# Drehrumbum/viterbi.dll

Measured on AMD Instinct MI355X. Metric: decoded Mbit/s per GPU on batched 768-bit DAB FIC frames; bit-exact vs AVX2 ref, higher is better.
Workload: dtype u8

## Files before the change

viterbi.dll_amd/csrc/rs_dev.h:

```cpp
#pragma once
#include "vit_internal.h"

namespace {

constexpr int NN = 255;
constexpr int NROOTS = 10;
constexpr int PADN = 135;
constexpr int NCW = 120, NMSG = 110;
constexpr int RS_THREADS = 256;
constexpr int ATO_ZERO = 512;
constexpr int ATO_SIZE = 768;
#ifndef COOP_MAX3
#define COOP_MAX3 12
#endif
#ifndef COOP_MAX5
#define COOP_MAX5 28
#endif

struct GfTables {
    uint8_t ato[ATO_SIZE];
    uint8_t iof[256];
};
constexpr GfTables make_tables() {
    GfTables t{};
    uint8_t alpha[256] = {};
    int sr = 1;
    t.iof[0] = NN;
    for (int i = 0; i < NN; i++) {
        t.iof[sr] = (uint8_t)i;
        alpha[i] = (uint8_t)sr;
        sr <<= 1;
        if (sr & 256) sr ^= 285;
        sr &= NN;
    }
    for (int i = 0; i < ATO_ZERO; i++) t.ato[i] = alpha[i % 255];
    return t;
}
__constant__ GfTables g_gf = make_tables();

struct QuadTable {
    uint8_t q[256];
};
constexpr QuadTable make_quad_table() {
    const GfTables t = make_tables();
    QuadTable Q{};
    for (int y = 2; y < 256; y++) {
        const int y2 = t.ato[(2 * t.iof[y]) % 255];
        const int c = y2 ^ y;
        if (Q.q[c] == 0) Q.q[c] = (uint8_t)y;
    }
    return Q;
}

#ifndef RS_LFSR2
#define RS_LFSR2 1
#endif
constexpr int NIB_TABLES = RS_LFSR2 ? 4 : 2;
struct NibTable {
    uint32_t w[NIB_TABLES * 16 * 4];
};
constexpr NibTable make_nib_table() {
    const GfTables t = make_tables();
    uint8_t g[NROOTS + 1] = {1};
    int deg = 0;
    for (int i = 0; i < NROOTS; i++) {
        const uint8_t root = t.ato[i];
        uint8_t ng[NROOTS + 1] = {};
        for (int j = 0; j <= deg; j++) {
            ng[j + 1] ^= g[j];
            if (g[j]) ng[j] ^= t.ato[t.iof[g[j]] + t.iof[root]];
        }
        deg++;
        for (int j = 0; j <= deg; j++) g[j] = ng[j];
    }
    NibTable G{};
    for (int half = 0; half < 2; half++)
        for (int n = 1; n < 16; n++) {
            const int x = half ? n << 4 : n;
            for (int j = 0; j < NROOTS; j++) {
                const uint32_t prod = g[j] ? t.ato[t.iof[x] + t.iof[g[j]]] : 0u;
                G.w[(half * 16 + n) * 4 + (j < 8 ? j / 4 : 3)] |= prod << (8 * (j % 4));
            }
        }
#if RS_LFSR2
    for (int half = 0; half < 2; half++)
        for (int n = 1; n < 16; n++) {
            const int x = half ? n << 4 : n;
            for (int j = 0; j < NROOTS; j++) {
                uint8_t c = j ? g[j - 1] : 0;
                if (g[9] && g[j]) c ^= t.ato[t.iof[g[9]] + t.iof[g[j]]];
                const uint32_t prod = c ? t.ato[t.iof[x] + t.iof[c]] : 0u;
                G.w[((2 + half) * 16 + n) * 4 + (j < 8 ? j / 4 : 3)] |= prod << (8 * (j % 4));
            }
        }
#endif
    return G;
}
__constant__ NibTable g_nib = make_nib_table();
__constant__ QuadTable g_quad = make_quad_table();

constexpr int STEP_TERMS = 5;
struct StepTable {
    uint32_t w[STEP_TERMS * 256];
};
constexpr StepTable make_step_table() {
    const GfTables t = make_tables();
    StepTable S{};
    for (int j = 1; j <= STEP_TERMS; j++)
        for (int c = 1; c < 256; c++)
            for (int k = 1; k <= 4; k++) S.w[(j - 1) * 256 + c] |= (uint32_t)t.ato[t.iof[c] + j * k] << (8 * (k - 1));
    return S;
}
__constant__ StepTable g_step = make_step_table();

typedef uint32_t u32x4 __attribute__((ext_vector_type(4)));
#define LDS __attribute__((address_space(3)))
__device__ __forceinline__ uint32_t xor3(uint32_t a, uint32_t b, uint32_t c) { return __builtin_amdgcn_bitop3_b32(a, b, c, 0x96); }
__device__ __forceinline__ uint32_t mod255(uint32_t x) { return (x * 0x1010102u) >> 24; }
__device__ __forceinline__ uint32_t mod510(uint32_t x) { return x < x - NN ? x : x - NN; }

__device__ __forceinline__ int chien_log(const uint32_t (&lam)[NROOTS + 1], bool need, int deg_lambda, uint8_t* col,
                                         uint32_t stride, const uint8_t* __restrict__ ato) {
    uint32_t b[NROOTS + 1], live[NROOTS + 1];
#pragma unroll
    for (int j = 1; j <= NROOTS; j++) {
        live[j] = need && lam[j] != NN ? 0xFFu : 0u;
        b[j] = live[j] ? lam[j] : 0u;
    }
    bool searching = need;
    int count = 0;
    for (int i = 1; i <= NN; i++) {
        if (searching) {
            uint32_t q = 1;
#pragma unroll
            for (int j = 1; j <= NROOTS; j++) {
                b[j] += (uint32_t)j;
                b[j] = b[j] < (uint32_t)NN ? b[j] : b[j] - NN;
                q ^= ato[b[j]] & live[j];
            }
            if (q == 0) {
                col[(uint32_t)(NMSG + count) * stride] = (uint8_t)i;
                if (++count == deg_lambda) searching = false;
            }
        }
        if (!__any(searching)) break;
    }
    return count;
}

template <int D>
__device__ __forceinline__ int chien_quad(const uint32_t (&lam)[NROOTS + 1], bool need, uint8_t* col, uint32_t stride,
                                          const uint8_t* __restrict__ ato, const uint32_t* __restrict__ step) {
    static_assert(D <= STEP_TERMS, "step table");
    uint32_t adr[D + 1];
#pragma unroll
    for (int j = 1; j <= D; j++) adr[j] = need && lam[j] != NN ? (uint32_t)ato[lam[j]] << 2 : 0u;
    int count = 0;
    for (int blk = 0; blk < 8; blk++) {
        uint32_t m = 0;
#pragma unroll
        for (int it = 0; it < 8; it++) {
            uint32_t q = 0x01010101u;
#pragma unroll
            for (int j = 1; j <= D; j++) {
                const uint32_t t =
                    *reinterpret_cast<const uint32_t*>(reinterpret_cast<const uint8_t*>(step) + (j - 1) * 1024 + adr[j]);
                q ^= t;
                adr[j] = (t >> 22) & 0x3FCu;
            }
            const uint32_t z = ~(((q & 0x7F7F7F7Fu) + 0x7F7F7F7Fu) | q | 0x7F7F7F7Fu);
            m = (m >> 1) | z;
        }
        if (blk == 7) m &= 0x7FFFFFFFu;
        if (__any(m != 0)) {
            while (m) {
                const uint32_t bit = (uint32_t)__ffs((int)m) - 1u;
                m &= m - 1u;
                col[(uint32_t)(NMSG + count) * stride] = (uint8_t)(32u * blk + 4u * (bit & 7u) + (bit >> 3) + 1u);
                count++;
            }
        }
    }
    return count;
}

template <int D>
__device__ __forceinline__ void chien_wave(const uint32_t (&lam)[NROOTS + 1], bool need, bool failed, int deg_lambda,
                                           uint32_t sfid, int& count, bool& dropped, uint8_t* cwbase, uint32_t coloff,
                                           uint32_t stride, const uint8_t* __restrict__ ato,
                                           const uint32_t* __restrict__ step) {
    static_assert(D <= STEP_TERMS, "step table");
    const uint32_t lane = __lane_id();
    uint32_t e[D + 1], lgz[D + 1];
#pragma unroll
    for (int j = 1; j <= D; j++) {
        e[j] = mod255(4u * (uint32_t)j * lane);
        lgz[j] = lam[j] == (uint32_t)NN ? (uint32_t)ATO_ZERO : lam[j];
    }
    const uint32_t keep = lane == 63u ? 0x7FFFFFFFu : 0xFFFFFFFFu;
    const uint64_t failm = __ballot(failed);
    uint64_t work = __ballot(need) | failm;
    uint64_t gone = 0;
    while (work) {
        const int owner = __builtin_ctzll(work);
        work &= work - 1;
        bool fail = true;
        if (!((failm >> owner) & 1u)) {
            uint32_t q = 0x01010101u;
#pragma unroll
            for (int j = 1; j <= D; j++) {
                const uint32_t c = ato[(uint32_t)__builtin_amdgcn_readlane(lgz[j], owner) + e[j]];
                q ^= step[(j - 1) * 256 + c];
            }
            uint32_t z = ~(((q & 0x7F7F7F7Fu) + 0x7F7F7F7Fu) | q | 0x7F7F7F7Fu) & keep;
            uint8_t* ocol = cwbase + __builtin_amdgcn_readlane(coloff, owner);
            uint32_t found = 0;
            uint64_t hit;
            while ((hit = __ballot(z != 0)) != 0) {
                if (z) {
                    const uint32_t below =
                        __builtin_amdgcn_mbcnt_hi((uint32_t)(hit >> 32), __builtin_amdgcn_mbcnt_lo((uint32_t)hit, 0u));
                    const uint32_t k = ((uint32_t)__ffs((int)z) - 1u) >> 3;
                    ocol[__umul24(NMSG + found + below, stride)] = (uint8_t)(4u * lane + k + 1u);
                    z &= z - 1u;
                }
                found += (uint32_t)__popcll(hit);
            }
            if (lane == (uint32_t)owner) count = (int)found;
            fail = (int)found != __builtin_amdgcn_readlane(deg_lambda, owner);
        }
        if (fail) {
            const uint64_t later = __ballot(sfid == (uint32_t)__builtin_amdgcn_readlane(sfid, owner)) & ~((2ull << owner) - 1ull);
            work &= ~later;
            gone |= later;
        }
    }
    dropped = (gone >> lane) & 1u;
}

__device__ int rs_correct(uint32_t (&s)[NROOTS], bool err, uint32_t sfid, uint8_t* cwbase, uint32_t coloff,
                          uint32_t stride, const uint8_t* __restrict__ ato, const uint8_t* __restrict__ iof,
                          const uint8_t* __restrict__ qsol, const uint32_t* __restrict__ step) {
    uint8_t* const col = cwbase + coloff;
    uint32_t lam[NROOTS + 1];
#pragma unroll
    for (int i = 0; i <= NROOTS; i++) lam[i] = NN;
    int deg_lambda = 0;
    if (err) {
#pragma unroll
        for (int i = 0; i < NROOTS; i++) s[i] = iof[s[i]];

        uint32_t pl[NROOTS + 1], b[NROOTS + 1];
#pragma unroll
        for (int i = 0; i <= NROOTS; i++) { pl[i] = 0; b[i] = NN; }
        pl[0] = 1;
        lam[0] = 0;
        b[0] = 0;
        int el = 0;
        bool geo = s[0] != NN && s[1] != NN;
        const uint32_t lr = mod510(s[1] + NN - s[0]);
        uint32_t expect = s[1];
#pragma unroll
        for (int i = 2; i < NROOTS; i++) {
            expect = mod510(expect + lr);
            geo = geo && s[i] == expect;
        }
        const bool shortcut = __all(geo);
        if (shortcut) lam[1] = lr;
#pragma unroll
        for (int r = 1; r <= NROOTS; r++) {
            if (shortcut) break;
            uint32_t discr = 0;
#pragma unroll
            for (int i = 0; i < r; i++) {
                const bool term = lam[i] != NN && s[r - i - 1] != NN;
                if (__any(term)) {
                    if (term) discr ^= ato[lam[i] + s[r - i - 1]];
                }
            }
            discr = iof[discr];
            const bool zero = discr == NN;
            if (__any(!zero)) {
                const bool grow = !zero && 2 * el <= r - 1;
                uint32_t t[NROOTS + 1];
#pragma unroll
                for (int i = 0; i < r; i++) {
                    t[i + 1] = pl[i + 1];
                    if (!zero && b[i] != NN) t[i + 1] ^= ato[discr + b[i]];
                }
                if (grow) el = r - el;
#pragma unroll
                for (int i = r; i >= 0; i--) {
                    const uint32_t scaled = lam[i] == NN ? (uint32_t)NN : mod510(lam[i] + NN - discr);
                    const uint32_t shifted = i ? b[i - 1] : (uint32_t)NN;
                    b[i] = grow ? scaled : shifted;
                }
#pragma unroll
                for (int i = 1; i <= r; i++) {
                    pl[i] = zero ? pl[i] : t[i];
                    lam[i] = iof[pl[i]];
                }
            } else {
#pragma unroll
                for (int i = r; i > 0; i--) b[i] = b[i - 1];
                b[0] = NN;
            }
        }
#pragma unroll
        for (int i = 0; i <= NROOTS; i++)
            if (lam[i] != NN) deg_lambda = i;
    }
    int dmax = 0;
#pragma unroll
    for (int d = 1; d <= NROOTS; d++)
        if (__any(deg_lambda >= d)) dmax = d;
    dmax = __builtin_amdgcn_readfirstlane(dmax);

    uint32_t root[NROOTS];
#pragma unroll
    for (int k = 0; k < NROOTS; k++) root[k] = 0;
    int count = 0;
    if (deg_lambda == 1) {
        root[0] = (uint32_t)NN - lam[1];
        count = 1;
    } else if (dmax >= 2 && deg_lambda == 2) {
        if (lam[1] != NN) {
            const uint32_t y0 = qsol[ato[mod255(lam[2] + 2u * (NN - lam[1]))]];
            if (y0) {
                const uint32_t scale = lam[1] + NN - lam[2];
                uint32_t r0 = mod255(scale + iof[y0]), r1 = mod255(scale + iof[y0 ^ 1u]);
                r0 = r0 ? r0 : (uint32_t)NN;
                r1 = r1 ? r1 : (uint32_t)NN;
                root[0] = r0 < r1 ? r0 : r1;
                root[1] = r0 < r1 ? r1 : r0;
                count = 2;
            }
        } else {
            count = 1;
        }
    }
    bool dropped = false;
    if (dmax >= 3) {
        const bool need = deg_lambda >= 3;
        if (dmax <= STEP_TERMS) {
            const int heavy = __popcll(__ballot(need));
            if (heavy <= (dmax <= 3 ? COOP_MAX3 : COOP_MAX5)) {
                const bool failed = err && !need && deg_lambda != count;
                if (dmax <= 3) chien_wave<3>(lam, need, failed, deg_lambda, sfid, count, dropped, cwbase, coloff, stride, ato, step);
                else chien_wave<STEP_TERMS>(lam, need, failed, deg_lambda, sfid, count, dropped, cwbase, coloff, stride, ato, step);
            } else {
                const int found = dmax <= 3 ? chien_quad<3>(lam, need, col, stride, ato, step)
                                            : chien_quad<STEP_TERMS>(lam, need, col, stride, ato, step);
                if (need) count = found;
            }
        } else if (need) {
            count = chien_log(lam, need, deg_lambda, col, stride, ato);
        }
        if (need && !dropped) {
#pragma unroll
            for (int k = 0; k < NROOTS; k++)
                if (k < dmax && k < count) root[k] = col[(uint32_t)(NMSG + k) * stride];
        }
    }
    if (!err || dropped) return 0;
    if (deg_lambda != count) return -1;

    const int deg_omega = deg_lambda - 1;
    uint32_t om[NROOTS];
#pragma unroll
    for (int i = 0; i < NROOTS; i++) {
        om[i] = NN;
        if (i < dmax) {
            uint32_t tmp = 0;
#pragma unroll
            for (int j = 0; j <= i; j++)
                if (s[i - j] != NN && lam[j] != NN) tmp ^= ato[s[i - j] + lam[j]];
            om[i] = i <= deg_omega ? (uint32_t)iof[tmp] : (uint32_t)NN;
        }
    }
    const int top = (deg_lambda < NROOTS - 1 ? deg_lambda : NROOTS - 1) & ~1;
#pragma unroll
    for (int j = NROOTS - 1; j >= 0; j--) {
        if (j >= dmax) continue;
        const uint32_t rt = root[j];
        if (j < count && rt >= PADN + 1) {
            uint32_t num1 = 0;
#pragma unroll
            for (int i = 0; i < NROOTS; i++)
                if (i < dmax && i <= deg_omega && om[i] != NN) num1 ^= ato[mod255(om[i] + i * rt)];
            if (num1) {
                const uint32_t num2 = ato[NN - rt];
                uint32_t den = 0;
#pragma unroll
                for (int i = 0; i < NROOTS; i += 2)
                    if (i < dmax && i <= top && lam[i + 1] != NN) den ^= ato[mod255(lam[i + 1] + i * rt)];
                const uint32_t tmp = (uint32_t)iof[num1] + iof[num2] + (NN - iof[den]);
                col[(rt - 1 - PADN) * stride] ^= ato[mod255(tmp)];
            }
        }
    }
    return count;
}

__device__ int decode_rs(bool active, uint32_t sfid, uint8_t* cw, uint32_t tid, const uint8_t* __restrict__ ato,
                         const uint8_t* __restrict__ iof, const uint8_t* __restrict__ mulp,
                         const uint8_t* __restrict__ qsol, const uint32_t* __restrict__ step) {
    uint32_t s[NROOTS];
    uint32_t syn = 0;
    if (active) {
        const uint8_t* col = cw + tid;
        const uint32_t d0 = col[0];
#pragma unroll
        for (int i = 0; i < NROOTS; i++) s[i] = d0;
        for (int j = 1; j < NCW; j++) {
            const uint32_t d = col[j * RS_THREADS];
            s[0] ^= d;
#pragma unroll
            for (int i = 1; i < NROOTS; i++) s[i] = d ^ mulp[i * 256 + s[i]];
        }
#pragma unroll
        for (int i = 0; i < NROOTS; i++) syn |= s[i];
    }
    if (!__any(syn != 0)) return 0;
    return rs_correct(s, syn != 0, sfid, cw, tid, RS_THREADS, ato, iof, qsol, step);
}

__device__ int decode_rs_lfsr(bool active, uint32_t sfid, uint8_t* cwbase, uint32_t coloff, uint32_t stride,
                              const uint8_t* __restrict__ ato, const uint8_t* __restrict__ iof,
                              const uint8_t* __restrict__ qsol, const uint32_t* __restrict__ gnib,
                              const uint32_t* __restrict__ step) {
    uint32_t r0 = 0, r1 = 0, r2 = 0;
    const uint8_t* q = cwbase + coloff;
    const uint32_t nibbase = (uint32_t)(uintptr_t)(const LDS uint32_t*)gnib;
#if RS_LFSR2
    static_assert(NCW % 2 == 0, "two data bytes per step");
#pragma unroll 4
    for (int k = 0; k < NCW; k += 2, q += 2 * stride) {
        const uint32_t d1 = q[0], d2 = q[stride];
        const uint32_t a4 = r2 >> 4;
        const u32x4 lo2 = *reinterpret_cast<const LDS u32x4*>(nibbase + 512u + (a4 & 0xF0u));
        const u32x4 hi2 = *reinterpret_cast<const LDS u32x4*>(nibbase + 768u + ((a4 >> 4) & 0xF0u));
        const u32x4 lo1 = *reinterpret_cast<const LDS u32x4*>(nibbase + ((r2 << 4) & 0xF0u));
        const u32x4 hi1 = *reinterpret_cast<const LDS u32x4*>(nibbase + 256u + (r2 & 0xF0u));
        r2 = xor3(xor3(__builtin_amdgcn_alignbit(r2, r1, 16), lo1.w, hi1.w), lo2.w, hi2.w);
        r1 = xor3(xor3(__builtin_amdgcn_alignbit(r1, r0, 16), lo1.y, hi1.y), lo2.y, hi2.y);
        r0 = xor3(xor3((((r0 << 16) | d2) | (d1 << 8)), lo1.x, hi1.x), lo2.x, hi2.x);
        asm volatile("" ::"v"(lo1.z), "v"(hi1.z), "v"(lo2.z), "v"(hi2.z));
    }
#else
#pragma unroll 8
    for (int k = 0; k < NCW; k++, q += stride) {
#ifdef RS_DIAG_NO_DATA
        const uint32_t d = (uint32_t)k;
#else
        const uint32_t d = *q;
#endif
#ifdef RS_DIAG_FAKE_IDX
        const uint32_t f4 = (uint32_t)k << 4;
#else
        const uint32_t f4 = r2 >> 4;
#endif
        const u32x4 lo = *reinterpret_cast<const LDS u32x4*>(nibbase + (f4 & 0xF0u));
        const u32x4 hi = *reinterpret_cast<const LDS u32x4*>(nibbase + 256u + ((f4 >> 4) & 0xF0u));
        r2 = xor3(__builtin_amdgcn_alignbit(r2, r1, 24), lo.w, hi.w);
        r1 = xor3(__builtin_amdgcn_alignbit(r1, r0, 24), lo.y, hi.y);
        r0 = xor3((r0 << 8) | d, lo.x, hi.x);
        asm volatile("" ::"v"(lo.z), "v"(hi.z));
    }
#endif
    r2 &= 0xFFFFu;
    const bool err = active && (r0 | r1 | r2) != 0;
    if (!__any(err)) return 0;
    uint32_t s[NROOTS];
    if (err) {
        uint32_t lg[NROOTS];
        s[0] = 0;
#pragma unroll
        for (int j = 0; j < NROOTS; j++) {
            const uint32_t c = ((j < 4 ? r0 : j < 8 ? r1 : r2) >> (8 * (j & 3))) & 0xFFu;
            s[0] ^= c;
            lg[j] = c ? (uint32_t)iof[c] : (uint32_t)ATO_ZERO;
        }
#pragma unroll
        for (int i = 1; i < NROOTS; i++) {
            uint32_t v = 0;
#pragma unroll
            for (int j = 0; j < NROOTS; j++) v ^= ato[lg[j] + (uint32_t)(i * j)];
            s[i] = v;
            if (i % 3 == 0) __builtin_amdgcn_sched_barrier(0);
        }
    }
    return rs_correct(s, err, sfid, cwbase, coloff, stride, ato, iof, qsol, step);
}

template <typename V>
__device__ __forceinline__ void copy_vec(uint8_t* dst, const uint8_t* src, uint32_t n, uint32_t tid) {
    const uint32_t nv = n / (uint32_t)sizeof(V);
#pragma clang loop vectorize(disable) interleave(disable)
    for (uint32_t i = tid; i < nv; i += RS_THREADS) reinterpret_cast<V*>(dst)[i] = reinterpret_cast<const V*>(src)[i];
#pragma clang loop vectorize(disable) interleave(disable)
    for (uint32_t i = nv * (uint32_t)sizeof(V) + tid; i < n; i += RS_THREADS) dst[i] = src[i];
}
__device__ __attribute__((noinline)) void copy_linear(uint8_t* dst, const uint8_t* src, uint32_t n, uint32_t tid) {
    const uintptr_t a = reinterpret_cast<uintptr_t>(dst) | reinterpret_cast<uintptr_t>(src);
    if ((a & 15u) == 0) copy_vec<uint4>(dst, src, n, tid);
    else if ((a & 7u) == 0) copy_vec<uint2>(dst, src, n, tid);
    else if ((a & 3u) == 0) copy_vec<uint32_t>(dst, src, n, tid);
    else copy_vec<uint8_t>(dst, src, n, tid);
}

template <typename V>
__device__ __forceinline__ void copy_out(uint8_t* dst0, const uint8_t* cw, const int* s_minfail, uint32_t nloc,
                                         uint32_t in_sz, uint32_t out_sz, uint32_t tid) {
    const uint32_t wps = out_sz / (uint32_t)sizeof(V);
    uint32_t l = tid / wps, o = tid - l * wps;
    while (l < nloc) {
        if (s_minfail[l] == 0x7FFFFFFF)
            reinterpret_cast<V*>(dst0 + l * out_sz)[o] = reinterpret_cast<const V*>(cw + l * in_sz)[o];
        o += RS_THREADS;
        while (o >= wps) {
            o -= wps;
            l++;
        }
    }
}

}
```

viterbi.dll_amd/csrc/rs_kernels.hip:

```cpp
#include "rs_dev.h"

namespace {

__global__ __launch_bounds__(RS_THREADS) void rs_kernel_wide(const uint8_t* __restrict__ p, uint8_t* __restrict__ out,
                                                        int32_t* __restrict__ ret, uint32_t rsdims,
                                                        long long nsf) {
    __shared__ uint8_t cw[NCW * RS_THREADS];
    __shared__ uint8_t ato[ATO_SIZE];
    __shared__ uint8_t iof[256];
    __shared__ uint8_t mulp[(NROOTS + 1) * 256];
    __shared__ uint8_t qsol[256];
    __shared__ uint32_t step[STEP_TERMS * 256];
    __shared__ int s_minfail[RS_THREADS];
    __shared__ int s_sum[RS_THREADS];
    __shared__ int s_fail[RS_THREADS];
    const int tid = threadIdx.x;
    for (int i = tid; i < ATO_SIZE; i += RS_THREADS) ato[i] = g_gf.ato[i];
    iof[tid] = g_gf.iof[tid];
    qsol[tid] = g_quad.q[tid];
    for (int i = 0; i <= NROOTS; i++) mulp[i * 256 + tid] = tid ? g_gf.ato[g_gf.iof[tid] + i] : 0;
    for (int i = tid; i < STEP_TERMS * 256; i += RS_THREADS) step[i] = g_step.w[i];
    __syncthreads();

    const uint32_t spb = rsdims <= RS_THREADS ? RS_THREADS / rsdims : 1u;
    const uint32_t nchunk = rsdims <= RS_THREADS ? 1u : (rsdims + RS_THREADS - 1) / RS_THREADS;
    const long long ngroups = (nsf + spb - 1) / spb;
    const size_t in_sz = (size_t)NCW * rsdims, out_sz = (size_t)NMSG * rsdims;

    for (long long g = blockIdx.x; g < ngroups; g += gridDim.x) {
        const uint32_t lsf = rsdims <= RS_THREADS ? tid / rsdims : 0u;
        const uint32_t lsfc = lsf < spb ? lsf : 0u;
        const long long sf = g * spb + lsf;
        if (tid < (int)spb) {
            s_sum[tid] = 0;
            s_fail[tid] = 0;
        }
        __syncthreads();
        for (uint32_t ch = 0; ch < nchunk; ch++) {
            if (tid < (int)spb) s_minfail[tid] = 0x7FFFFFFF;
            __syncthreads();
            const uint32_t colidx = rsdims <= RS_THREADS ? tid - lsf * rsdims : ch * RS_THREADS + tid;
            const bool active = lsf < spb && sf < nsf && colidx < rsdims && !s_fail[lsfc];
            if (active) {
                const uint8_t* src = p + (size_t)sf * in_sz + colidx;
                for (int k = 0; k < NCW; k++) cw[k * RS_THREADS + tid] = src[(size_t)k * rsdims];
            }
            const int res = decode_rs(active, lsf, cw, tid, ato, iof, mulp, qsol, step);
            if (res < 0) atomicMin(&s_minfail[lsf], (int)colidx);
            __syncthreads();
            const int mf = s_minfail[lsfc];
            if (active && (int)colidx < mf) {
                uint8_t* dst = out + (size_t)sf * out_sz + colidx;
                for (int k = 0; k < NMSG; k++) dst[(size_t)k * rsdims] = cw[k * RS_THREADS + tid];
                atomicAdd(&s_sum[lsf], res);
            }
            __syncthreads();
            if (tid < (int)spb && s_minfail[tid] != 0x7FFFFFFF) s_fail[tid] = 1;
            __syncthreads();
        }
        if (tid < (int)spb && g * spb + tid < nsf) ret[g * spb + tid] = s_fail[tid] ? -1 : s_sum[tid];
        __syncthreads();
    }
}


__global__ __launch_bounds__(RS_THREADS, 4) void rs_kernel(const uint8_t* __restrict__ p, uint8_t* __restrict__ out,
                                                        int32_t* __restrict__ ret, uint32_t rsdims,
                                                        long long nsf, int host_polls_ret) {
    __shared__ __attribute__((aligned(16))) uint8_t cw[NCW * RS_THREADS];
    __shared__ __attribute__((aligned(256))) uint32_t gnib[NIB_TABLES * 16 * 4];
    __shared__ uint32_t step[STEP_TERMS * 256];
    __shared__ uint8_t ato[ATO_SIZE];
    __shared__ uint8_t iof[256];
    __shared__ uint8_t qsol[256];
    __shared__ int s_minfail[RS_THREADS];
    __shared__ int s_sum[RS_THREADS];
    const uint32_t tid = threadIdx.x;
    for (uint32_t i = tid; i < ATO_SIZE; i += RS_THREADS) ato[i] = g_gf.ato[i];
    iof[tid] = g_gf.iof[tid];
    qsol[tid] = g_quad.q[tid];
    if (tid < (uint32_t)NIB_TABLES * 16u * 4u) gnib[tid] = g_nib.w[tid];
    for (uint32_t i = tid; i < STEP_TERMS * 256u; i += RS_THREADS) step[i] = g_step.w[i];
    __syncthreads();

    const uint32_t spb = RS_THREADS / rsdims;
    const long long ngroups = (nsf + spb - 1) / spb;
    const uint32_t in_sz = NCW * rsdims, out_sz = NMSG * rsdims;
    const uint32_t lsf = tid / rsdims, colidx = tid - lsf * rsdims;
    constexpr int NOFAIL = 0x7FFFFFFF;

    constexpr uint32_t PRE = NCW * RS_THREADS / 8u / RS_THREADS;
    const bool pre_ok = (reinterpret_cast<uintptr_t>(p) & 7u) == 0;
    uint2 pre[PRE];
    auto prefetch = [&](long long gg) {
        const long long s0 = gg * spb;
        const uint32_t nl = nsf - s0 < (long long)spb ? (uint32_t)(nsf - s0) : spb;
        const uint32_t nw = nl * in_sz / 8u;
        const uint2* src = reinterpret_cast<const uint2*>(p + (size_t)s0 * in_sz);
#pragma unroll
        for (uint32_t k = 0; k < PRE; k++) {
            const uint32_t i = tid + k * RS_THREADS;
            pre[k] = i < nw ? src[i] : make_uint2(0u, 0u);
        }
    };
    if (pre_ok && (long long)blockIdx.x < ngroups) prefetch(blockIdx.x);

#ifndef RS_PRIO_ROT
#define RS_PRIO_ROT 1
#endif
#if RS_PRIO_ROT
    uint32_t rs_slot, rs_pass = 0;
    {
        uint32_t hwid;
        asm volatile("s_getreg_b32 %0, hwreg(HW_REG_HW_ID)" : "=s"(hwid));
        rs_slot = hwid & 3u;
#if RS_PRIO_ROT == 2
        __shared__ uint32_t s_slot;
        if (tid == 0) s_slot = rs_slot;
        __syncthreads();
        rs_slot = s_slot;
        rs_slot = (uint32_t)__builtin_amdgcn_readfirstlane((int)rs_slot);
#endif
    }
#endif
    for (long long g = blockIdx.x; g < ngroups; g += gridDim.x) {
#if RS_PRIO_ROT
        if (ngroups > 2 * (long long)gridDim.x)
        switch ((rs_slot + rs_pass) & 3u) {
            case 0: __builtin_amdgcn_s_setprio(0); break;
            case 1: __builtin_amdgcn_s_setprio(1); break;
            case 2: __builtin_amdgcn_s_setprio(2); break;
            default: __builtin_amdgcn_s_setprio(3); break;
        }
        rs_pass++;
#endif
        const long long sf0 = g * spb;
        const uint32_t nloc = nsf - sf0 < (long long)spb ? (uint32_t)(nsf - sf0) : spb;
        if (tid < spb) {
            s_minfail[tid] = NOFAIL;
            s_sum[tid] = 0;
        }
        if (pre_ok) {
            const uint32_t nw = nloc * in_sz / 8u;
#pragma unroll
            for (uint32_t k = 0; k < PRE; k++) {
                const uint32_t i = tid + k * RS_THREADS;
                if (i < nw) reinterpret_cast<uint2*>(cw)[i] = pre[k];
            }
            if (g + gridDim.x < ngroups) prefetch(g + gridDim.x);
        } else {
            copy_linear(cw, p + (size_t)sf0 * in_sz, nloc * in_sz, tid);
        }
        __syncthreads();
        const bool active = lsf < nloc;
        const int res = decode_rs_lfsr(active, lsf, cw, active ? lsf * in_sz + colidx : 0u, rsdims, ato, iof, qsol, gnib, step);
        if (res < 0) atomicMin(&s_minfail[lsf], (int)colidx);
        __syncthreads();
        uint8_t* dst0 = out + (size_t)sf0 * out_sz;
        if ((out_sz & 3u) == 0 && (reinterpret_cast<uintptr_t>(dst0) & 3u) == 0) {
            if ((out_sz & 15u) == 0 && (in_sz & 15u) == 0 && (reinterpret_cast<uintptr_t>(dst0) & 15u) == 0)
                copy_out<uint4>(dst0, cw, s_minfail, nloc, in_sz, out_sz, tid);
            else
                copy_out<uint32_t>(dst0, cw, s_minfail, nloc, in_sz, out_sz, tid);
            if (active) {
                const int mf = s_minfail[lsf];
                if (mf != NOFAIL && (int)colidx < mf) {
                    uint8_t* dst = dst0 + (lsf * out_sz + colidx);
                    const uint8_t* src = cw + lsf * in_sz + colidx;
#pragma clang loop vectorize(disable) interleave(disable)
                    for (int k = 0; k < NMSG; k++) dst[(size_t)k * rsdims] = src[k * rsdims];
                }
                if ((int)colidx < mf) atomicAdd(&s_sum[lsf], res);
            }
        } else if (active) {
            const int mf = s_minfail[lsf];
            if ((int)colidx < mf) {
                uint8_t* dst = dst0 + (lsf * out_sz + colidx);
                const uint8_t* src = cw + lsf * in_sz + colidx;
#pragma clang loop vectorize(disable) interleave(disable)
                for (int k = 0; k < NMSG; k++) dst[(size_t)k * rsdims] = src[k * rsdims];
                atomicAdd(&s_sum[lsf], res);
            }
        }
        if (host_polls_ret) __threadfence_system();
        __syncthreads();
        if (tid < nloc) {
            const int32_t r = s_minfail[tid] != NOFAIL ? -1 : s_sum[tid];
            if (host_polls_ret) __hip_atomic_store(&ret[sf0 + tid], r, __ATOMIC_RELEASE, __HIP_MEMORY_SCOPE_SYSTEM);
            else ret[sf0 + tid] = r;
        }
        __syncthreads();
    }
}

}

hipError_t rs_launch(const uint8_t* d_p, uint8_t* d_out, int32_t* d_ret, uint32_t rsdims, int64_t nsf,
                     hipStream_t stream, bool host_polls_ret) {
    if (nsf <= 0 || rsdims == 0) return hipSuccess;
    if (host_polls_ret && (nsf != 1 || rsdims > RS_THREADS)) return hipErrorInvalidValue;
    const uint32_t spb = rsdims <= RS_THREADS ? RS_THREADS / rsdims : 1u;
    long long groups = (nsf + spb - 1) / spb;
    if (groups > (1 << 20)) groups = 1 << 20;
    if (rsdims <= RS_THREADS) {
        int dev = 0;
        const int cus = hipGetDevice(&dev) == hipSuccess ? vit_device_cus(dev) : 256;
        const long long resident = 4LL * cus;
        if (groups > resident) groups = resident;
    }
    if (rsdims <= RS_THREADS)
        hipLaunchKernelGGL(rs_kernel, dim3((unsigned)groups), dim3(RS_THREADS), 0, stream, d_p, d_out, d_ret, rsdims,
                           (long long)nsf, host_polls_ret ? 1 : 0);
    else
        hipLaunchKernelGGL(rs_kernel_wide, dim3((unsigned)groups), dim3(RS_THREADS), 0, stream, d_p, d_out, d_ret,
                           rsdims, (long long)nsf);
    return hipGetLastError();
}
```

viterbi.dll_amd/csrc/rs_table.hip:

```cpp
#include "rs_dev.h"

namespace {

__device__ __forceinline__ void rs_pass_finish(uint8_t* cw, uint32_t tid, uint32_t rsdims, uint32_t lsf, uint32_t colidx,
                                               uint32_t in_sz, uint32_t out_sz, uint32_t nloc, uint8_t* dst0, int32_t* ret0,
                                               const uint8_t* ato, const uint8_t* iof, const uint8_t* qsol, const uint32_t* gnib,
                                               const uint32_t* step, int* s_minfail, int* s_sum) {
    constexpr int NOFAIL = 0x7FFFFFFF;
    const bool active = lsf < nloc;
    const int res = decode_rs_lfsr(active, lsf, cw, active ? lsf * in_sz + colidx : 0u, rsdims, ato, iof, qsol, gnib, step);
    if (res < 0) atomicMin(&s_minfail[lsf], (int)colidx);
    __syncthreads();
    if ((out_sz & 3u) == 0 && (reinterpret_cast<uintptr_t>(dst0) & 3u) == 0) {
        if ((out_sz & 15u) == 0 && (in_sz & 15u) == 0 && (reinterpret_cast<uintptr_t>(dst0) & 15u) == 0)
            copy_out<uint4>(dst0, cw, s_minfail, nloc, in_sz, out_sz, tid);
        else
            copy_out<uint32_t>(dst0, cw, s_minfail, nloc, in_sz, out_sz, tid);
        if (active) {
            const int mf = s_minfail[lsf];
            if (mf != NOFAIL && (int)colidx < mf) {
                uint8_t* dst = dst0 + (lsf * out_sz + colidx);
                const uint8_t* src = cw + lsf * in_sz + colidx;
#pragma clang loop vectorize(disable) interleave(disable)
                for (int k = 0; k < NMSG; k++) dst[(size_t)k * rsdims] = src[k * rsdims];
            }
            if ((int)colidx < mf) atomicAdd(&s_sum[lsf], res);
        }
    } else if (active) {
        const int mf = s_minfail[lsf];
        if ((int)colidx < mf) {
            uint8_t* dst = dst0 + (lsf * out_sz + colidx);
            const uint8_t* src = cw + lsf * in_sz + colidx;
#pragma clang loop vectorize(disable) interleave(disable)
            for (int k = 0; k < NMSG; k++) dst[(size_t)k * rsdims] = src[k * rsdims];
            atomicAdd(&s_sum[lsf], res);
        }
    }
    __syncthreads();
    if (tid < nloc) ret0[tid] = s_minfail[tid] != NOFAIL ? -1 : s_sum[tid];
}

struct RsPass {
    uint32_t rsdims, sf0, nloc;
    uint64_t in_off, out_off;
    uint32_t rec;
};
__device__ __forceinline__ RsPass rs_table_pass(const VitEnsTable& tab, uint32_t g) {
    const uint32_t k = vit_ens_find<&VitEnsEntry::pass0>(tab, g);
    const VitEnsEntry& e = tab.e[k];
    const uint32_t nsf = (k + 1u < tab.nsub ? tab.e[k + 1u].rec0 : tab.nrec) - e.rec0;
    RsPass ps;
    ps.rsdims = e.rsdims;
    const uint32_t spb = RS_THREADS / ps.rsdims;
    ps.sf0 = (g - e.pass0) * spb;
    ps.nloc = nsf - ps.sf0 < spb ? nsf - ps.sf0 : spb;
    ps.in_off = e.work_off + (uint64_t)ps.sf0 * (NCW * ps.rsdims);
    ps.out_off = e.rs_off + (uint64_t)ps.sf0 * (NMSG * ps.rsdims);
    ps.rec = e.rec0 + ps.sf0;
    return ps;
}

__global__ __launch_bounds__(RS_THREADS, 4) void rs_table_kernel(const uint8_t* __restrict__ p, uint8_t* __restrict__ out,
                                                                 int32_t* __restrict__ ret, const VitEnsTable tab) {
    __shared__ __attribute__((aligned(16))) uint8_t cw[NCW * RS_THREADS];
    __shared__ __attribute__((aligned(256))) uint32_t gnib[NIB_TABLES * 16 * 4];
    __shared__ uint32_t step[STEP_TERMS * 256];
    __shared__ uint8_t ato[ATO_SIZE];
    __shared__ uint8_t iof[256];
    __shared__ uint8_t qsol[256];
    __shared__ int s_minfail[RS_THREADS];
    __shared__ int s_sum[RS_THREADS];
    const uint32_t tid = threadIdx.x;
    for (uint32_t i = tid; i < ATO_SIZE; i += RS_THREADS) ato[i] = g_gf.ato[i];
    iof[tid] = g_gf.iof[tid];
    qsol[tid] = g_quad.q[tid];
    if (tid < (uint32_t)NIB_TABLES * 16u * 4u) gnib[tid] = g_nib.w[tid];
    for (uint32_t i = tid; i < STEP_TERMS * 256u; i += RS_THREADS) step[i] = g_step.w[i];
    __syncthreads();

    constexpr int NOFAIL = 0x7FFFFFFF;
    constexpr uint32_t PRE = NCW * RS_THREADS / 8u / RS_THREADS;
    const bool pre_ok = (reinterpret_cast<uintptr_t>(p) & 7u) == 0;
    const uint32_t npass = tab.npass;
    uint2 pre[PRE];
    auto prefetch = [&](const RsPass& ps) {
        const uint32_t nw = ps.nloc * (NCW * ps.rsdims) / 8u;
        const uint2* src = reinterpret_cast<const uint2*>(p + ps.in_off);
#pragma unroll
        for (uint32_t k = 0; k < PRE; k++) {
            const uint32_t i = tid + k * RS_THREADS;
            pre[k] = i < nw ? src[i] : make_uint2(0u, 0u);
        }
    };
    RsPass next = {};
    if (blockIdx.x < npass) {
        next = rs_table_pass(tab, blockIdx.x);
        if (pre_ok) prefetch(next);
    }
#if RS_PRIO_ROT
    uint32_t rs_slot, rs_pass = 0;
    {
        uint32_t hwid;
        asm volatile("s_getreg_b32 %0, hwreg(HW_REG_HW_ID)" : "=s"(hwid));
        rs_slot = hwid & 3u;
    }
#endif
    for (uint32_t g = blockIdx.x; g < npass; g += gridDim.x) {
#if RS_PRIO_ROT
        if (npass > 2u * gridDim.x)
        switch ((rs_slot + rs_pass) & 3u) {
            case 0: __builtin_amdgcn_s_setprio(0); break;
            case 1: __builtin_amdgcn_s_setprio(1); break;
            case 2: __builtin_amdgcn_s_setprio(2); break;
            default: __builtin_amdgcn_s_setprio(3); break;
        }
        rs_pass++;
#endif
        const RsPass ps = next;
        const uint32_t rsdims = ps.rsdims, in_sz = NCW * rsdims, out_sz = NMSG * rsdims;
        const uint32_t lsf = tid / rsdims, colidx = tid - lsf * rsdims;
        if (tid < RS_THREADS / rsdims) {
            s_minfail[tid] = NOFAIL;
            s_sum[tid] = 0;
        }
        const bool more = g + gridDim.x < npass;
        if (more) next = rs_table_pass(tab, g + gridDim.x);
        if (pre_ok) {
            const uint32_t nw = ps.nloc * in_sz / 8u;
#pragma unroll
            for (uint32_t k = 0; k < PRE; k++) {
                const uint32_t i = tid + k * RS_THREADS;
                if (i < nw) reinterpret_cast<uint2*>(cw)[i] = pre[k];
            }
            if (more) prefetch(next);
        } else {
            copy_linear(cw, p + ps.in_off, ps.nloc * in_sz, tid);
        }
        __syncthreads();
        rs_pass_finish(cw, tid, rsdims, lsf, colidx, in_sz, out_sz, ps.nloc, out + ps.out_off, ret + ps.rec, ato, iof, qsol, gnib,
                       step, s_minfail, s_sum);
        __syncthreads();
    }
}

}

hipError_t rs_table_launch(const uint8_t* d_work, uint8_t* d_rs_out, int32_t* d_ret, const VitEnsTable& tab, hipStream_t stream) {
    if (tab.npass == 0) return hipSuccess;
    int dev = 0;
    const unsigned resident = 4u * (unsigned)(hipGetDevice(&dev) == hipSuccess ? vit_device_cus(dev) : 256);
    hipLaunchKernelGGL(rs_table_kernel, dim3(tab.npass < resident ? tab.npass : resident), dim3(RS_THREADS), 0, stream, d_work,
                       d_rs_out, d_ret, tab);
    return hipGetLastError();
}
```

Baseline: 124,900.

## Widen RS syndrome LFSR to four bytes per trip and merge shared result slots

Generalises the nibble-table generation so the Reed-Solomon LFSR encoder-style remainder loop consumes four codeword bytes per iteration (eight nibble table lookups) instead of two, halving the serial loop-carried dependency chain length. It also packs the per-frame min-fail column and correction sum into one 32-bit LDS word to cut shared memory so a fourth workgroup fits per CU. The wider step doubles the LDS table size and per-trip lookups, and the 16-bit packing bounds correction counts.

```diff
diff --git a/viterbi.dll_amd/csrc/rs_dev.h b/viterbi.dll_amd/csrc/rs_dev.h
--- a/viterbi.dll_amd/csrc/rs_dev.h
+++ b/viterbi.dll_amd/csrc/rs_dev.h
@@ -52,10 +52,11 @@
     return Q;
 }
 
-#ifndef RS_LFSR2
-#define RS_LFSR2 1
-#endif
-constexpr int NIB_TABLES = RS_LFSR2 ? 4 : 2;
+#ifndef RS_LFSR_W
+#define RS_LFSR_W 4
+#endif
+static_assert(RS_LFSR_W == 1 || RS_LFSR_W == 2 || RS_LFSR_W == 4, "data bytes per LFSR trip");
+constexpr int NIB_TABLES = 2 * RS_LFSR_W;
 struct NibTable {
     uint32_t w[NIB_TABLES * 16 * 4];
 };
@@ -74,26 +75,22 @@
         for (int j = 0; j <= deg; j++) g[j] = ng[j];
     }
     NibTable G{};
-    for (int half = 0; half < 2; half++)
-        for (int n = 1; n < 16; n++) {
-            const int x = half ? n << 4 : n;
-            for (int j = 0; j < NROOTS; j++) {
-                const uint32_t prod = g[j] ? t.ato[t.iof[x] + t.iof[g[j]]] : 0u;
-                G.w[(half * 16 + n) * 4 + (j < 8 ? j / 4 : 3)] |= prod << (8 * (j % 4));
-            }
-        }
-#if RS_LFSR2
-    for (int half = 0; half < 2; half++)
-        for (int n = 1; n < 16; n++) {
-            const int x = half ? n << 4 : n;
-            for (int j = 0; j < NROOTS; j++) {
-                uint8_t c = j ? g[j - 1] : 0;
-                if (g[9] && g[j]) c ^= t.ato[t.iof[g[9]] + t.iof[g[j]]];
-                const uint32_t prod = c ? t.ato[t.iof[x] + t.iof[c]] : 0u;
-                G.w[((2 + half) * 16 + n) * 4 + (j < 8 ? j / 4 : 3)] |= prod << (8 * (j % 4));
-            }
-        }
-#endif
+    for (int tb = 0; tb < RS_LFSR_W; tb++)
+        for (int half = 0; half < 2; half++)
+            for (int n = 1; n < 16; n++) {
+                uint8_t r[NROOTS] = {}, sh[NROOTS] = {};
+                r[NROOTS - RS_LFSR_W + tb] = (uint8_t)(half ? n << 4 : n);
+                for (int j = 0; j + RS_LFSR_W < NROOTS; j++) sh[j + RS_LFSR_W] = r[j];
+                for (int s = 0; s < RS_LFSR_W; s++) {
+                    const uint8_t f = r[NROOTS - 1];
+                    for (int j = NROOTS - 1; j >= 0; j--) {
+                        const uint8_t fb = f && g[j] ? t.ato[t.iof[f] + t.iof[g[j]]] : (uint8_t)0;
+                        r[j] = (uint8_t)((j ? r[j - 1] : 0) ^ fb);
+                    }
+                }
+                for (int j = 0; j < NROOTS; j++)
+                    G.w[((2 * tb + half) * 16 + n) * 4 + (j < 8 ? j / 4 : 3)] |= (uint32_t)(r[j] ^ sh[j]) << (8 * (j % 4));
+            }
     return G;
 }
 __constant__ NibTable g_nib = make_nib_table();
@@ -115,7 +112,13 @@
 
 typedef uint32_t u32x4 __attribute__((ext_vector_type(4)));
 #define LDS __attribute__((address_space(3)))
-__device__ __forceinline__ uint32_t xor3(uint32_t a, uint32_t b, uint32_t c) { return __builtin_amdgcn_bitop3_b32(a, b, c, 0x96); }
+__host__ __device__ __forceinline__ uint32_t xor3(uint32_t a, uint32_t b, uint32_t c) {
+#ifdef __HIP_DEVICE_COMPILE__
+    return __builtin_amdgcn_bitop3_b32(a, b, c, 0x96);
+#else
+    return a ^ b ^ c;
+#endif
+}
 __device__ __forceinline__ uint32_t mod255(uint32_t x) { return (x * 0x1010102u) >> 24; }
 __device__ __forceinline__ uint32_t mod510(uint32_t x) { return x < x - NN ? x : x - NN; }
 
@@ -425,6 +428,27 @@
     return rs_correct(s, syn != 0, sfid, cw, tid, RS_THREADS, ato, iof, qsol, step);
 }
 
+template <typename Row>
+__host__ __device__ __forceinline__ void lfsr4_trip(uint32_t& r0, uint32_t& r1, uint32_t& r2, uint32_t d1, uint32_t d2,
+                                                    uint32_t d3, uint32_t d4, Row row) {
+    const uint32_t a4 = r2 >> 4, b4 = r1 >> 12;
+    const u32x4 lo9 = row(1536u + (a4 & 0xF0u));
+    const u32x4 hi9 = row(1792u + ((a4 >> 4) & 0xF0u));
+    const u32x4 lo8 = row(1024u + ((r2 << 4) & 0xF0u));
+    const u32x4 hi8 = row(1280u + (r2 & 0xF0u));
+    const u32x4 lo7 = row(512u + ((b4 >> 8) & 0xF0u));
+    const u32x4 hi7 = row(768u + ((b4 >> 12) & 0xF0u));
+    const u32x4 lo6 = row(b4 & 0xF0u);
+    const u32x4 hi6 = row(256u + ((b4 >> 4) & 0xF0u));
+    const uint32_t d = (((d1 << 8 | d2) << 8 | d3) << 8) | d4;
+    r2 = xor3(xor3(xor3(xor3(r1, lo9.w, hi9.w), lo8.w, hi8.w), lo7.w, hi7.w), lo6.w, hi6.w);
+    r1 = xor3(xor3(xor3(xor3(r0, lo9.y, hi9.y), lo8.y, hi8.y), lo7.y, hi7.y), lo6.y, hi6.y);
+    r0 = xor3(xor3(xor3(xor3(d, lo9.x, hi9.x), lo8.x, hi8.x), lo7.x, hi7.x), lo6.x, hi6.x);
+#ifdef __HIP_DEVICE_COMPILE__
+    asm volatile("" ::"v"(lo9.z), "v"(hi9.z), "v"(lo8.z), "v"(hi8.z), "v"(lo7.z), "v"(hi7.z), "v"(lo6.z), "v"(hi6.z));
+#endif
+}
+
 __device__ int decode_rs_lfsr(bool active, uint32_t sfid, uint8_t* cwbase, uint32_t coloff, uint32_t stride,
                               const uint8_t* __restrict__ ato, const uint8_t* __restrict__ iof,
                               const uint8_t* __restrict__ qsol, const uint32_t* __restrict__ gnib,
@@ -432,8 +456,15 @@
     uint32_t r0 = 0, r1 = 0, r2 = 0;
     const uint8_t* q = cwbase + coloff;
     const uint32_t nibbase = (uint32_t)(uintptr_t)(const LDS uint32_t*)gnib;
-#if RS_LFSR2
-    static_assert(NCW % 2 == 0, "two data bytes per step");
+#if RS_LFSR_W == 4
+    static_assert(NCW % 4 == 0, "four data bytes per trip");
+#pragma unroll 2
+    for (int k = 0; k < NCW; k += 4, q += 4 * stride) {
+        const uint32_t d1 = q[0], d2 = q[stride], d3 = q[2 * stride], d4 = q[3 * stride];
+        lfsr4_trip(r0, r1, r2, d1, d2, d3, d4, [nibbase](uint32_t off) { return *reinterpret_cast<const LDS u32x4*>(nibbase + off); });
+    }
+#elif RS_LFSR_W == 2
+    static_assert(NCW % 2 == 0, "two data bytes per trip");
 #pragma unroll 4
     for (int k = 0; k < NCW; k += 2, q += 2 * stride) {
         const uint32_t d1 = q[0], d2 = q[stride];
@@ -509,13 +540,17 @@
     else copy_vec<uint8_t>(dst, src, n, tid);
 }
 
+constexpr uint32_t RES_NOFAIL = 0xFFFFu;
+constexpr uint32_t RES_CLEAR = RES_NOFAIL << 16;
+constexpr size_t RS_LDS_BUDGET = 160 * 1024 / 4;
+static_assert(RS_THREADS * NROOTS < 65536 && RS_THREADS <= RES_NOFAIL, "a pass's corrections and column indices fit 16 bits");
 template <typename V>
-__device__ __forceinline__ void copy_out(uint8_t* dst0, const uint8_t* cw, const int* s_minfail, uint32_t nloc,
+__device__ __forceinline__ void copy_out(uint8_t* dst0, const uint8_t* cw, const uint32_t* s_res, uint32_t nloc,
                                          uint32_t in_sz, uint32_t out_sz, uint32_t tid) {
     const uint32_t wps = out_sz / (uint32_t)sizeof(V);
     uint32_t l = tid / wps, o = tid - l * wps;
     while (l < nloc) {
-        if (s_minfail[l] == 0x7FFFFFFF)
+        if (s_res[l] >= RES_CLEAR)
             reinterpret_cast<V*>(dst0 + l * out_sz)[o] = reinterpret_cast<const V*>(cw + l * in_sz)[o];
         o += RS_THREADS;
         while (o >= wps) {
diff --git a/viterbi.dll_amd/csrc/rs_kernels.hip b/viterbi.dll_amd/csrc/rs_kernels.hip
--- a/viterbi.dll_amd/csrc/rs_kernels.hip
+++ b/viterbi.dll_amd/csrc/rs_kernels.hip
@@ -73,13 +73,14 @@
     __shared__ uint8_t ato[ATO_SIZE];
     __shared__ uint8_t iof[256];
     __shared__ uint8_t qsol[256];
-    __shared__ int s_minfail[RS_THREADS];
-    __shared__ int s_sum[RS_THREADS];
+    __shared__ uint32_t s_res[RS_THREADS];
+    static_assert(sizeof(cw) + sizeof(gnib) + sizeof(step) + sizeof(ato) + sizeof(iof) + sizeof(qsol) + sizeof(s_res) <= RS_LDS_BUDGET,
+                  "the fourth workgroup of a CU");
     const uint32_t tid = threadIdx.x;
     for (uint32_t i = tid; i < ATO_SIZE; i += RS_THREADS) ato[i] = g_gf.ato[i];
     iof[tid] = g_gf.iof[tid];
     qsol[tid] = g_quad.q[tid];
-    if (tid < (uint32_t)NIB_TABLES * 16u * 4u) gnib[tid] = g_nib.w[tid];
+    for (uint32_t i = tid; i < (uint32_t)NIB_TABLES * 16u * 4u; i += RS_THREADS) gnib[i] = g_nib.w[i];
     for (uint32_t i = tid; i < STEP_TERMS * 256u; i += RS_THREADS) step[i] = g_step.w[i];
     __syncthreads();
 
@@ -87,7 +88,6 @@
     const long long ngroups = (nsf + spb - 1) / spb;
     const uint32_t in_sz = NCW * rsdims, out_sz = NMSG * rsdims;
     const uint32_t lsf = tid / rsdims, colidx = tid - lsf * rsdims;
-    constexpr int NOFAIL = 0x7FFFFFFF;
 
     constexpr uint32_t PRE = NCW * RS_THREADS / 8u / RS_THREADS;
     const bool pre_ok = (reinterpret_cast<uintptr_t>(p) & 7u) == 0;
@@ -136,10 +136,7 @@
 #endif
         const long long sf0 = g * spb;
         const uint32_t nloc = nsf - sf0 < (long long)spb ? (uint32_t)(nsf - sf0) : spb;
-        if (tid < spb) {
-            s_minfail[tid] = NOFAIL;
-            s_sum[tid] = 0;
-        }
+        if (tid < spb) s_res[tid] = RES_CLEAR;
         if (pre_ok) {
             const uint32_t nw = nloc * in_sz / 8u;
 #pragma unroll
@@ -154,38 +151,38 @@
         __syncthreads();
         const bool active = lsf < nloc;
         const int res = decode_rs_lfsr(active, lsf, cw, active ? lsf * in_sz + colidx : 0u, rsdims, ato, iof, qsol, gnib, step);
-        if (res < 0) atomicMin(&s_minfail[lsf], (int)colidx);
+        if (res < 0) atomicMin(&s_res[lsf], colidx << 16);
         __syncthreads();
         uint8_t* dst0 = out + (size_t)sf0 * out_sz;
         if ((out_sz & 3u) == 0 && (reinterpret_cast<uintptr_t>(dst0) & 3u) == 0) {
             if ((out_sz & 15u) == 0 && (in_sz & 15u) == 0 && (reinterpret_cast<uintptr_t>(dst0) & 15u) == 0)
-                copy_out<uint4>(dst0, cw, s_minfail, nloc, in_sz, out_sz, tid);
+                copy_out<uint4>(dst0, cw, s_res, nloc, in_sz, out_sz, tid);
             else
-                copy_out<uint32_t>(dst0, cw, s_minfail, nloc, in_sz, out_sz, tid);
+                copy_out<uint32_t>(dst0, cw, s_res, nloc, in_sz, out_sz, tid);
             if (active) {
-                const int mf = s_minfail[lsf];
-                if (mf != NOFAIL && (int)colidx < mf) {
+                const uint32_t mf = s_res[lsf] >> 16;
+                if (mf != RES_NOFAIL && colidx < mf) {
                     uint8_t* dst = dst0 + (lsf * out_sz + colidx);
                     const uint8_t* src = cw + lsf * in_sz + colidx;
 #pragma clang loop vectorize(disable) interleave(disable)
                     for (int k = 0; k < NMSG; k++) dst[(size_t)k * rsdims] = src[k * rsdims];
                 }
-                if ((int)colidx < mf) atomicAdd(&s_sum[lsf], res);
+                if (colidx < mf) atomicAdd(&s_res[lsf], (uint32_t)res);
             }
         } else if (active) {
-            const int mf = s_minfail[lsf];
-            if ((int)colidx < mf) {
+            const uint32_t mf = s_res[lsf] >> 16;
+            if (colidx < mf) {
                 uint8_t* dst = dst0 + (lsf * out_sz + colidx);
                 const uint8_t* src = cw + lsf * in_sz + colidx;
 #pragma clang loop vectorize(disable) interleave(disable)
                 for (int k = 0; k < NMSG; k++) dst[(size_t)k * rsdims] = src[k * rsdims];
-                atomicAdd(&s_sum[lsf], res);
+                atomicAdd(&s_res[lsf], (uint32_t)res);
             }
         }
         if (host_polls_ret) __threadfence_system();
         __syncthreads();
         if (tid < nloc) {
-            const int32_t r = s_minfail[tid] != NOFAIL ? -1 : s_sum[tid];
+            const int32_t r = s_res[tid] < RES_CLEAR ? -1 : (int32_t)(s_res[tid] & 0xFFFFu);
             if (host_polls_ret) __hip_atomic_store(&ret[sf0 + tid], r, __ATOMIC_RELEASE, __HIP_MEMORY_SCOPE_SYSTEM);
             else ret[sf0 + tid] = r;
         }
diff --git a/viterbi.dll_amd/csrc/rs_table.hip b/viterbi.dll_amd/csrc/rs_table.hip
--- a/viterbi.dll_amd/csrc/rs_table.hip
+++ b/viterbi.dll_amd/csrc/rs_table.hip
@@ -5,39 +5,38 @@
 __device__ __forceinline__ void rs_pass_finish(uint8_t* cw, uint32_t tid, uint32_t rsdims, uint32_t lsf, uint32_t colidx,
                                                uint32_t in_sz, uint32_t out_sz, uint32_t nloc, uint8_t* dst0, int32_t* ret0,
                                                const uint8_t* ato, const uint8_t* iof, const uint8_t* qsol, const uint32_t* gnib,
-                                               const uint32_t* step, int* s_minfail, int* s_sum) {
-    constexpr int NOFAIL = 0x7FFFFFFF;
+                                               const uint32_t* step, uint32_t* s_res) {
     const bool active = lsf < nloc;
     const int res = decode_rs_lfsr(active, lsf, cw, active ? lsf * in_sz + colidx : 0u, rsdims, ato, iof, qsol, gnib, step);
-    if (res < 0) atomicMin(&s_minfail[lsf], (int)colidx);
+    if (res < 0) atomicMin(&s_res[lsf], colidx << 16);
     __syncthreads();
     if ((out_sz & 3u) == 0 && (reinterpret_cast<uintptr_t>(dst0) & 3u) == 0) {
         if ((out_sz & 15u) == 0 && (in_sz & 15u) == 0 && (reinterpret_cast<uintptr_t>(dst0) & 15u) == 0)
-            copy_out<uint4>(dst0, cw, s_minfail, nloc, in_sz, out_sz, tid);
+            copy_out<uint4>(dst0, cw, s_res, nloc, in_sz, out_sz, tid);
         else
-            copy_out<uint32_t>(dst0, cw, s_minfail, nloc, in_sz, out_sz, tid);
+            copy_out<uint32_t>(dst0, cw, s_res, nloc, in_sz, out_sz, tid);
         if (active) {
-            const int mf = s_minfail[lsf];
-            if (mf != NOFAIL && (int)colidx < mf) {
+            const uint32_t mf = s_res[lsf] >> 16;
+            if (mf != RES_NOFAIL && colidx < mf) {
                 uint8_t* dst = dst0 + (lsf * out_sz + colidx);
                 const uint8_t* src = cw + lsf * in_sz + colidx;
 #pragma clang loop vectorize(disable) interleave(disable)
                 for (int k = 0; k < NMSG; k++) dst[(size_t)k * rsdims] = src[k * rsdims];
             }
-            if ((int)colidx < mf) atomicAdd(&s_sum[lsf], res);
+            if (colidx < mf) atomicAdd(&s_res[lsf], (uint32_t)res);
         }
     } else if (active) {
-        const int mf = s_minfail[lsf];
-        if ((int)colidx < mf) {
+        const uint32_t mf = s_res[lsf] >> 16;
+        if (colidx < mf) {
             uint8_t* dst = dst0 + (lsf * out_sz + colidx);
             const uint8_t* src = cw + lsf * in_sz + colidx;
 #pragma clang loop vectorize(disable) interleave(disable)
             for (int k = 0; k < NMSG; k++) dst[(size_t)k * rsdims] = src[k * rsdims];
-            atomicAdd(&s_sum[lsf], res);
+            atomicAdd(&s_res[lsf], (uint32_t)res);
         }
     }
     __syncthreads();
-    if (tid < nloc) ret0[tid] = s_minfail[tid] != NOFAIL ? -1 : s_sum[tid];
+    if (tid < nloc) ret0[tid] = s_res[tid] < RES_CLEAR ? -1 : (int32_t)(s_res[tid] & 0xFFFFu);
 }
 
 struct RsPass {
@@ -68,17 +67,17 @@
     __shared__ uint8_t ato[ATO_SIZE];
     __shared__ uint8_t iof[256];
     __shared__ uint8_t qsol[256];
-    __shared__ int s_minfail[RS_THREADS];
-    __shared__ int s_sum[RS_THREADS];
+    __shared__ uint32_t s_res[RS_THREADS];
+    static_assert(sizeof(cw) + sizeof(gnib) + sizeof(step) + sizeof(ato) + sizeof(iof) + sizeof(qsol) + sizeof(s_res) <= RS_LDS_BUDGET,
+                  "the fourth workgroup of a CU");
     const uint32_t tid = threadIdx.x;
     for (uint32_t i = tid; i < ATO_SIZE; i += RS_THREADS) ato[i] = g_gf.ato[i];
     iof[tid] = g_gf.iof[tid];
     qsol[tid] = g_quad.q[tid];
-    if (tid < (uint32_t)NIB_TABLES * 16u * 4u) gnib[tid] = g_nib.w[tid];
+    for (uint32_t i = tid; i < (uint32_t)NIB_TABLES * 16u * 4u; i += RS_THREADS) gnib[i] = g_nib.w[i];
     for (uint32_t i = tid; i < STEP_TERMS * 256u; i += RS_THREADS) step[i] = g_step.w[i];
     __syncthreads();
 
-    constexpr int NOFAIL = 0x7FFFFFFF;
     constexpr uint32_t PRE = NCW * RS_THREADS / 8u / RS_THREADS;
     const bool pre_ok = (reinterpret_cast<uintptr_t>(p) & 7u) == 0;
     const uint32_t npass = tab.npass;
@@ -119,10 +118,7 @@
         const RsPass ps = next;
         const uint32_t rsdims = ps.rsdims, in_sz = NCW * rsdims, out_sz = NMSG * rsdims;
         const uint32_t lsf = tid / rsdims, colidx = tid - lsf * rsdims;
-        if (tid < RS_THREADS / rsdims) {
-            s_minfail[tid] = NOFAIL;
-            s_sum[tid] = 0;
-        }
+        if (tid < RS_THREADS / rsdims) s_res[tid] = RES_CLEAR;
         const bool more = g + gridDim.x < npass;
         if (more) next = rs_table_pass(tab, g + gridDim.x);
         if (pre_ok) {
@@ -138,7 +134,7 @@
         }
         __syncthreads();
         rs_pass_finish(cw, tid, rsdims, lsf, colidx, in_sz, out_sz, ps.nloc, out + ps.out_off, ret + ps.rec, ato, iof, qsol, gnib,
-                       step, s_minfail, s_sum);
+                       step, s_res);
         __syncthreads();
     }
 }
```

Measured after the change: 124,100. About the same (-0.6%).
